# xiyichen/smplify-x-partial

Hardware: AMD Instinct MI355X
Metric: fitted frames/sec (higher is better)
Workload: dtype f32; 1 GPU; configs[1]: 256 synthetic frames/GPU, body-only K=25, camera + 5-stage L-BFGS (fit_smplx_smplifyx.yaml, use_vposer=False); frames_per_gpu=256, lbs_mode=dense, gemm_columns_per_gpu=256, parallelism=frames sharded, dp1, closure_evals_per_frame_max=4429, non_finite=0

## Files before the change

include/sfx.h:

```cpp
#ifndef SFX_H_
#define SFX_H_
#include <stdint.h>

#ifdef __cplusplus
extern "C" {
#endif

typedef struct sfx_model sfx_model;
typedef struct sfx_batch sfx_batch;

typedef struct sfx_model_desc {
    int32_t V, F, J;
    int32_t num_betas, num_expr;
    int32_t num_pca;
    const float*   v_template;
    const float*   shapedirs;
    const float*   posedirs;
    const float*   J_regressor;
    const float*   lbs_weights;
    const int32_t* parents;
    const float*   hands_comp_l;
    const float*   hands_comp_r;
    const float*   pose_mean;
    const int32_t* faces;
// ... 95 lines not shown
                          const float* reye, const float* pose_embedding,
                          const float* regression_pose);
int  sfx_batch_get_params(sfx_batch* b, float* cam_translation, float* global_orient,
                          float* betas, float* lhand, float* rhand, float* expression,
                          float* jaw, float* leye, float* reye, float* pose_embedding,
                          float* body_pose );

int  sfx_batch_num_vars(sfx_batch* b, int32_t stage);
int  sfx_batch_closure(sfx_batch* b, int32_t stage, float* loss_out, float* grad_out, void* stream);

int  sfx_batch_guess_init(sfx_batch* b, const int32_t* pairs , int32_t n_pairs,
                          void* stream);

int  sfx_batch_fit(sfx_batch* b, int32_t first_stage, int32_t last_stage, void* stream);

int  sfx_batch_step(sfx_batch* b, int32_t stage, int32_t resume, float* loss_out, void* stream);

int  sfx_batch_get_grad(sfx_batch* b, int32_t stage, float* grad_out);

int  sfx_batch_pen_stats(sfx_batch* b, int32_t* stats_host , int32_t* ext_n_host );
int  sfx_batch_pen_flags(sfx_batch* b, int32_t* flags_host);
int  sfx_batch_pen_launches(sfx_batch* b);
int  sfx_batch_pen_pairs(sfx_batch* b, int32_t column, int32_t cap, int32_t* pairs_host, int32_t* n_out);

int  sfx_batch_get_stats(sfx_batch* b, float* stage_loss, int32_t* stage_evals,
                         int32_t* stage_ref_evals);

int  sfx_batch_trace(sfx_batch* b, int32_t capacity);
int  sfx_batch_get_trace(sfx_batch* b, float* records, int32_t* counts);

// ... 55 lines not shown
```

smplify-x-partial_amd/_capi.py:

```python
import ctypes as C
import os

import numpy as np

_HERE = os.path.dirname(os.path.abspath(__file__))
LIB_PATH = os.environ.get("SFX_LIB", os.path.join(_HERE, "libsfx.so"))
_lib = None

f32p = C.POINTER(C.c_float)
i32p = C.POINTER(C.c_int32)
f64p = C.POINTER(C.c_double)


class ModelDesc(C.Structure):
    _fields_ = [
        ("V", C.c_int32), ("F", C.c_int32), ("J", C.c_int32),
        ("num_betas", C.c_int32), ("num_expr", C.c_int32), ("num_pca", C.c_int32),
        ("v_template", f32p), ("shapedirs", f32p), ("posedirs", f32p), ("J_regressor", f32p),
        ("lbs_weights", f32p), ("parents", i32p), ("hands_comp_l", f32p), ("hands_comp_r", f32p),
        ("pose_mean", f32p), ("faces", i32p),
        ("n_extra", C.c_int32), ("extra_vertex_ids", i32p),
        ("n_lmk", C.c_int32), ("lmk_faces_idx", i32p), ("lmk_bary", f32p),
        ("n_dyn_rows", C.c_int32), ("n_dyn", C.c_int32), ("dyn_lmk_faces_idx", i32p), ("dyn_lmk_bary", f32p),
        ("K", C.c_int32), ("joint_map", i32p),
# ... 41 lines not shown
SYMBOLS = {
    "sfx_model_create": (C.c_int, [C.POINTER(ModelDesc), C.POINTER(C.c_void_p)]),
    "sfx_model_destroy": (None, [C.c_void_p]),
    "sfx_model_set_parts": (C.c_int, [C.c_void_p, i32p, i32p, i32p, C.c_int32]),
    "sfx_model_set_vposer": (C.c_int, [C.c_void_p, C.c_int32, C.c_int32] + [f32p] * 6),
    "sfx_lbs_forward": (C.c_int, [C.c_void_p, C.c_int32] + [C.c_void_p] * 12 + [C.c_void_p]),
    "sfx_batch_create": (C.c_int, [C.c_void_p, C.POINTER(BatchCfg), C.POINTER(StageWeights), C.POINTER(C.c_void_p)]),
    "sfx_batch_destroy": (None, [C.c_void_p]),
    "sfx_batch_set_frames": (C.c_int, [C.c_void_p] + [f32p] * 5),
    "sfx_batch_set_params": (C.c_int, [C.c_void_p] + [f32p] * 11),
    "sfx_batch_get_params": (C.c_int, [C.c_void_p] + [f32p] * 11),
    "sfx_batch_num_vars": (C.c_int, [C.c_void_p, C.c_int32]),
    "sfx_batch_closure": (C.c_int, [C.c_void_p, C.c_int32, f32p, f32p, C.c_void_p]),
    "sfx_batch_guess_init": (C.c_int, [C.c_void_p, i32p, C.c_int32, C.c_void_p]),
    "sfx_batch_fit": (C.c_int, [C.c_void_p, C.c_int32, C.c_int32, C.c_void_p]),
    "sfx_batch_step": (C.c_int, [C.c_void_p, C.c_int32, C.c_int32, f32p, C.c_void_p]),
    "sfx_batch_pen_stats": (C.c_int, [C.c_void_p, i32p, i32p]),
    "sfx_batch_get_grad": (C.c_int, [C.c_void_p, C.c_int32, f32p]),
    "sfx_batch_set_stage_weights_f64": (C.c_int, [C.c_void_p, C.POINTER(StageWeights64)]),
    "sfx_batch_set_frames_f64": (C.c_int, [C.c_void_p] + [f64p] * 5),
    "sfx_batch_set_params_f64": (C.c_int, [C.c_void_p] + [f64p] * 11),
    "sfx_batch_get_params_f64": (C.c_int, [C.c_void_p] + [f64p] * 11),
    "sfx_batch_closure_f64": (C.c_int, [C.c_void_p, C.c_int32, f64p, f64p, C.c_void_p]),
    "sfx_batch_get_grad_f64": (C.c_int, [C.c_void_p, C.c_int32, f64p]),
    "sfx_batch_get_stats": (C.c_int, [C.c_void_p, f32p, i32p, i32p]),
    "sfx_lbfgs_two_loop": (C.c_int, [C.c_void_p, C.c_void_p, C.c_int32, C.c_int32, C.c_void_p, C.c_void_p]),
    "sfx_batch_trace": (C.c_int, [C.c_void_p, C.c_int32]),
    "sfx_batch_get_trace": (C.c_int, [C.c_void_p, f32p, i32p]),
    "sfx_batch_forward": (C.c_int, [C.c_void_p, C.c_void_p, C.c_void_p, C.c_void_p]),
    "sfx_pen_create": (C.c_int, [C.c_int32, C.c_int32, i32p, i32p, i32p, i32p, C.c_int32, C.c_int32, C.c_int32,
# ... 111 lines not shown
```

smplify-x-partial_amd/csrc/api.hip:

```cpp
#include "../../include/sfx.h"
#include "sfx_internal.h"
#include "model_tables.h"

#include <algorithm>
#include <chrono>
#include <cmath>
#include <cstdarg>
#include <cstdio>
#include <cstring>
#include <map>
#include <memory>
#include <mutex>
#include <string>
#include <vector>

static thread_local char g_err[1024] = "";
void sfx_set_error(const char* fmt, ...) {
    va_list ap; va_start(ap, fmt); vsnprintf(g_err, sizeof(g_err), fmt, ap); va_end(ap);
}
extern "C" const char* sfx_last_error(void) { return g_err; }
extern "C" const char* sfx_version(void) { return "sfx 0.1.0 (gfx950)"; }

struct ProfAcc { double ms = 0; int64_t n = 0, seen = 0; double units = 0; std::vector<std::pair<hipEvent_t, hipEvent_t>> pend; };
static int g_prof = 0;
// ... 83 lines not shown
    DevModel M{};
    DevAlloc mem;
    std::vector<int> faces_host, segm_host, parents_host, ign_host;
    int NB = 0, NE = 0, NPCA = 0;
    std::vector<int> meta_host;
    sfx_batch* fwd = nullptr;
    int fwd_B = 0;
    sfx_pen* pen_idle = nullptr;
    int pen_idle_cols = 0, pen_idle_cap = 0, pen_idle_gen = -1;
    int parts_gen = 0;
    std::mutex pen_mu;
    ~sfx_model() { sfx_batch_destroy(fwd); sfx_pen_destroy(pen_idle); }
};

#define SFX_POLL_BUFS 8
struct sfx_batch {
    sfx_model* m = nullptr;
    BatchDev D{};
    DevAlloc mem;
    VarList* vl_dev = nullptr;
    StageW* sw_dev = nullptr;
    VarList vl_host[2];
    int* stage_host = nullptr;
    int* map_host = nullptr;
    int* act_dev = nullptr;
    int* act_new_dev = nullptr;
    int slots = 0;
    hipEvent_t poll_ev[SFX_POLL_BUFS] = {};
    std::vector<int> slot_host;
    int K = 0;
    sfx_pen* pen = nullptr;
    float pen_sigma = 0.f; int pen_outside = 1;
    int pen_cols = 0, pen_cap = 0, pen_gen = -1;
    std::map<int, hipGraphExec_t> pen_graphs;
    int pen_graph_nodes = 0;
    hipStream_t cap_stream = nullptr;
    int* pen_stats_all = nullptr;
    bool pen_chunked = false;
    bool f64 = false;
    StageW64* sw64_dev = nullptr;
    DevAlloc trace_mem;
    long long* dbg_buf = nullptr;
    ~sfx_batch() {
        for (auto& kv : pen_graphs) hipGraphExecDestroy(kv.second);
        if (cap_stream) hipStreamDestroy(cap_stream);
        if (pen) {
            (void)hipDeviceSynchronize();
            std::lock_guard<std::mutex> lk(m->pen_mu);
            if (pen_gen == m->parts_gen && (!m->pen_idle || m->pen_idle_cols <= pen_cols)) {
                sfx_pen_destroy(m->pen_idle);
                m->pen_idle = pen; m->pen_idle_cols = pen_cols; m->pen_idle_cap = pen_cap; m->pen_idle_gen = pen_gen;
            } else sfx_pen_destroy(pen);
        }
        if (stage_host) hipHostFree(stage_host);
        if (map_host) hipHostFree(map_host);
        for (hipEvent_t e : poll_ev) if (e) hipEventDestroy(e);
    }
};

static int refuse_f64(const sfx_batch* b, const char* fn) {
// ... 41 lines not shown
    M.J_template = mem.up(T.J_template); M.J_dirs = mem.up(T.J_dirs);
    M.J_template64 = mem.up(T.J_template64); M.J_dirs64 = mem.up(T.J_dirs64);
    M.comp_l = mem.up(d->hands_comp_l, (size_t)d->num_pca * SFX_NHAND); M.comp_r = mem.up(d->hands_comp_r, (size_t)d->num_pca * SFX_NHAND);
    M.pose_mean = mem.up(d->pose_mean, SFX_POSE);
    M.sj_start = mem.up(T.sj_start); M.sj_item = mem.up(T.sj_item); M.sj_w = mem.up(T.sj_w);
    M.dj_start = mem.up(T.dj_start); M.dj_item = mem.up(T.dj_item); M.dj_w = mem.up(T.dj_w);
    M.dynp_vid = mem.up(T.dynp_vid); M.dynp_w = mem.up(T.dynp_w); M.dynp_vt = mem.up(T.dynp_vt);
    M.dynp_wj = mem.up(T.dynp_wj); M.dynp_ww = mem.up(T.dynp_ww);
    M.dynp_js = T.dynp_js.empty() ? nullptr : mem.up(T.dynp_js);
    M.dynp_ji = mem.up(T.dynp_ji); M.dynp_jw = mem.up(T.dynp_jw);
    M.item_vid = mem.up(T.item_vid); M.item_w = mem.up(T.item_w);
    M.item_vt = mem.up(T.item_vt); M.item_wj = mem.up(T.item_wj); M.item_ww = mem.up(T.item_ww);
    M.dynp_us = T.dynp_us.empty() ? nullptr : mem.up(T.dynp_us);
    M.vslot = mem.up(T.vslot); M.item_uslot = mem.up(T.item_uslot);
    M.meta = mem.up(T.meta);
    m->meta_host = std::move(T.meta); m->faces_host = std::move(T.faces);
    if (mem.failed) { (void)hipGetLastError(); sfx_set_error("out of device memory (model constants)"); return -2; }
    if (hipDeviceSynchronize() != hipSuccess) { sfx_set_error("model upload failed"); return -2; }
    *out = m.release();
    return 0;
}

extern "C" void sfx_model_destroy(sfx_model* m) { delete m; }

extern "C" int sfx_model_set_parts(sfx_model* m, const int32_t* segm, const int32_t* parents, const int32_t* ign_pairs,
                                   int32_t n_ign) {
    if (!m) { sfx_set_error("null argument"); return -1; }
    { std::lock_guard<std::mutex> lk(m->pen_mu); ++m->parts_gen; if (m->pen_idle) { sfx_pen_destroy(m->pen_idle); m->pen_idle = nullptr; } }
    if (!segm && !parents) {
        m->segm_host.clear(); m->parents_host.clear(); m->ign_host.clear();
// ... 137 lines not shown
        D.cam64 = b->mem.zeros<double>((size_t)B * 8);
    }
    D.gt = b->mem.zeros<float>((size_t)B * K * 2);
    D.conf = b->mem.zeros<float>((size_t)B * K);
    D.jw = b->mem.zeros<float>((size_t)B * K);
    D.cmask = b->mem.zeros<float>((size_t)B * K);
    D.cam = b->mem.zeros<float>((size_t)B * 8);
    D.camR = b->mem.zeros<float>((size_t)B * 9);
    D.regpose = b->mem.zeros<float>((size_t)B * 63);
    D.fd = b->mem.zeros<float>((size_t)B * FD_N);
    D.f = b->mem.zeros<float>(B);
    D.g = b->mem.zeros<float>((size_t)B * SFX_NVAR_MAX);
    D.bodypose = b->mem.zeros<float>((size_t)B * 63);
    D.featR = b->mem.zeros<float>((size_t)SFX_KD_PAD * D.Bpad);
    D.AT = b->mem.zeros<float>((size_t)12 * SFX_JPAD * D.Bpad);
    D.verts = b->mem.zeros<float>((size_t)B * m->M.V * 3);
    D.fwd = b->mem.zeros<float>((size_t)B * SFX_FWD_N);
    D.uvp = b->mem.zeros<float>((size_t)B * std::max(1, m->M.n_uniq) * 3);
    if (D.cfg.pen) {
        const int F = (int)(m->faces_host.size() / 3);
        const bool parts = !m->segm_host.empty();
        const int pen_cols = (c->slots > 0 && c->slots < B && c->lbs_mode == 1) ? std::min(B, ((c->slots + 31) / 32) * 32) : B;
        const int pen_cap = std::max(1, c->max_collisions);
        {
            std::lock_guard<std::mutex> lk(m->pen_mu);
            if (m->pen_idle && m->pen_idle_cols >= pen_cols && m->pen_idle_cap == pen_cap && m->pen_idle_gen == m->parts_gen) {
                b->pen = m->pen_idle; b->pen_cols = m->pen_idle_cols;
                m->pen_idle = nullptr;
                sfx_pen_reuse(b->pen);
            } else if (m->pen_idle) { sfx_pen_destroy(m->pen_idle); m->pen_idle = nullptr; }
// ... 34 lines not shown
    D.stage_loss = b->mem.zeros<float>((size_t)B * (1 + SFX_MAX_STAGES));
    D.stage_evals = b->mem.zeros<int>((size_t)B * (1 + SFX_MAX_STAGES));
    D.stage_ref_evals = b->mem.zeros<int>((size_t)B * (1 + SFX_MAX_STAGES));
    D.X0 = b->mem.zeros<float>((size_t)B * SFX_NPAR_MAX);
    D.gocam = b->mem.zeros<float>((size_t)B * 4);
    D.stage_loss2 = b->mem.zeros<float>((size_t)B * (1 + SFX_MAX_STAGES));
    D.try_both = b->mem.zeros<int>(B);
    D.orient_pass = b->mem.zeros<int>(B);
    if (b->mem.failed) { (void)hipGetLastError(); sfx_set_error("out of device memory (batch of %d frames)", B); return -2; }
    if (hipHostMalloc((void**)&b->stage_host, (size_t)SFX_POLL_BUFS * B * sizeof(int)) != hipSuccess) b->stage_host = nullptr;
    if (hipHostMalloc((void**)&b->map_host, (size_t)SFX_POLL_BUFS * 3 * B * sizeof(int)) != hipSuccess) b->map_host = nullptr;
    if (c->lbs_mode == 1 && (!b->stage_host || !b->map_host)) {
        sfx_set_error("out of pinned host memory"); return -2; }
    for (int i = 0; i < SFX_POLL_BUFS; ++i)
        if (hipEventCreateWithFlags(&b->poll_ev[i], hipEventDisableTiming) != hipSuccess) { sfx_set_error("event creation failed"); return -2; }
    *out = b.release();
    return 0;
}

extern "C" void sfx_batch_destroy(sfx_batch* b) { delete b; }

__global__ void k_pack_fd(BatchDev D, int K) {
    const int b = blockIdx.x, t = threadIdx.x;
    float* fd = D.fd + (size_t)b * FD_N;
    for (int i = t; i < 2 * K; i += blockDim.x) fd[FD_GT + i] = D.gt[(size_t)b * K * 2 + i];
    for (int i = t; i < K; i += blockDim.x) {
        fd[FD_CONF + i] = D.conf[(size_t)b * K + i]; fd[FD_JW + i] = D.jw[(size_t)b * K + i]; fd[FD_CMASK + i] = D.cmask[(size_t)b * K + i]; }
    if (t < 8) fd[FD_CAM + t] = D.cam[(size_t)b * 8 + t];
    if (t < 9) fd[FD_CAMR + t] = D.camR[(size_t)b * 9 + t];
    if (t < 63) fd[FD_REG + t] = D.regpose[(size_t)b * 63 + t];
}
static void pack_fd(sfx_batch* b, hipStream_t s) {
    hipLaunchKernelGGL(k_pack_fd, dim3(b->D.cfg.B), dim3(128), 0, s, b->D, b->K);
}

// ... 450 lines not shown
        auto upload = [&](const std::vector<int>* fresh) -> int {
            int* h = b->map_host + (size_t)upl * 3 * B; upl = (upl + 1) % SFX_POLL_BUFS;
            memcpy(h, col.data(), (size_t)B * sizeof(int));
            memcpy(h + B, run.data(), run.size() * sizeof(int));
            SFX_CHECK(hipMemcpyAsync(D.slot, h, (size_t)B * sizeof(int), hipMemcpyHostToDevice, s));
            if (!run.empty()) SFX_CHECK(hipMemcpyAsync(b->act_dev, h + B, run.size() * sizeof(int), hipMemcpyHostToDevice, s));
            if (fresh && !fresh->empty()) {
                memcpy(h + 2 * B, fresh->data(), fresh->size() * sizeof(int));
                SFX_CHECK(hipMemcpyAsync(b->act_new_dev, h + 2 * B, fresh->size() * sizeof(int), hipMemcpyHostToDevice, s));
            }
            D.act = b->act_dev; D.nrun = (int)run.size();
            return 0;
        };
        D.nact = pool;
        if (int rc = upload(nullptr)) return rc;
        { ProfScope p("tick", s, D.nrun); launch_tick_dense(M, D, b->vl_dev, b->sw_dev, first_stage, last_stage, 0, s); }
        double host_enq_s = 0.0, host_wait_s = 0.0; long host_batches = 0;
        const double wall0 = std::chrono::duration<double>(std::chrono::steady_clock::now().time_since_epoch()).count();
        const int rpb = std::max(1, std::min(64, rpb_env > 0 ? rpb_env : 8));
        auto rounds = [&](int buf) -> int {
            if (dbg_nact) nact_hist[std::min(8, (D.nact - 1) / 32)] += rpb;
            const auto h0 = std::chrono::steady_clock::now();
            struct HostClock { const std::chrono::steady_clock::time_point t0; double& acc; long& n; bool on;
                               ~HostClock() { if (on) { acc += std::chrono::duration<double>(std::chrono::steady_clock::now() - t0).count(); ++n; } } } hc{h0, host_enq_s, host_batches, true};
            for (int q = 0; q < rpb; ++q, ++tick) {
                { ProfScope p("lbs_dense", s, D.nact); launch_lbs_dense(M, D, s); }
                if (int rc = eval_penetration(b, -2, s, true)) return rc;
                ProfScope p("tick", s, D.nrun);
                launch_tick_dense(M, D, b->vl_dev, b->sw_dev, first_stage, last_stage, 1, s);
            }
            SFX_CHECK(hipMemcpyAsync(b->stage_host + (size_t)buf * B, D.stage, (size_t)B * sizeof(int), hipMemcpyDeviceToHost, s));
            SFX_CHECK(hipEventRecord(b->poll_ev[buf], s));
            return 0;
        };
        const int ahead = std::max(1, std::min(SFX_POLL_BUFS - 1, ahead_env > 0 ? ahead_env : (b->pen ? 1 : 3)));
        long q_head = 0, q_next = 0;
        for (; q_next < ahead; ++q_next) if (int rc = rounds((int)(q_next % SFX_POLL_BUFS))) return rc;
        while (!done && tick < max_ticks + (long)rpb * (ahead + 1)) {
            if (int rc = rounds((int)(q_next % SFX_POLL_BUFS))) return rc;
            ++q_next;
            const int cur = (int)(q_head % SFX_POLL_BUFS); ++q_head;
            {
                const auto w0 = std::chrono::steady_clock::now();
                SFX_CHECK(hipEventSynchronize(b->poll_ev[cur]));
// ... 5 lines not shown
            bool changed = false;
            for (size_t r = 0; r < run.size(); ++r) {
                const int f = run[r];
                if (hq[f] <= last_stage) { run[w++] = f; continue; }
                changed = true;
                const int c = col[f];
                col[f] = -1;
                if (next_q < B) { const int nf = next_q++; col[nf] = c; fresh.push_back(nf); }
            }
            run.resize(w);
            for (int nf : fresh) run.push_back(nf);
            done = run.empty();
            if (!done && changed) {
                if (!fresh.empty()) {
                    if (int rc = upload(&fresh)) return rc;
                    BatchDev Dn = D; Dn.act = b->act_new_dev; Dn.nrun = (int)fresh.size();
                    ProfScope p("tick_admit", s, Dn.nrun);
                    launch_tick_dense(M, Dn, b->vl_dev, b->sw_dev, first_stage, last_stage, 0, s);
                } else if ((D.nact + 31) / 32 != ((int)run.size() + 31) / 32 || (D.nact > 16 && run.size() <= 16)) {
                    int q = 0;
                    for (int f : run) col[f] = q++;
                    D.nact = q;
                    if (int rc = upload(nullptr)) return rc;
                    ProfScope p("tick", s, D.nrun);
                    launch_tick_dense(M, D, b->vl_dev, b->sw_dev, first_stage, last_stage, 0, s);
                } else {
                    if (int rc = upload(nullptr)) return rc;
                }
            }
        }
        SFX_CHECK(hipStreamSynchronize(s));
        D.act = nullptr; D.nrun = 0;
        const double wall = std::chrono::duration<double>(std::chrono::steady_clock::now().time_since_epoch()).count() - wall0;
        {
            std::lock_guard<std::mutex> lk(g_prof_mu);
            g_loop_host[0] += host_enq_s; g_loop_host[1] += host_wait_s; g_loop_host[2] += wall; g_loop_host[3] += (double)host_batches * rpb;
        }
        if (dbg_host) {
            fprintf(stderr, "[sfx] host enqueue: %ld batches of rounds, %.1f us of host time per round, %.1f %% of the loop's %.1f ms wall time\n",
                    host_batches, 1e6 * host_enq_s / std::max(1L, host_batches * rpb), 100.0 * host_enq_s / std::max(wall, 1e-9), 1e3 * wall);
        }
        if (dbg_nact) {
            fprintf(stderr, "[sfx] rounds by active columns (<=32, <=64, ..., <=256, more), cumulative:");
            for (int i = 0; i < 9; ++i) fprintf(stderr, " %ld", nact_hist[i]);
            fprintf(stderr, "\n");
// ... 288 lines not shown
```

smplify-x-partial_amd/csrc/lbs_dense.hip:

```cpp
#include "sfx_internal.h"
#include <cstdlib>
#include <algorithm>

typedef float f32x4 __attribute__((ext_vector_type(4)));

#define DT 256
#ifndef KC
#define KC 32
#endif
#ifndef MINW
#define MINW 3
#endif
#define FB 128
#define VB 16
#define NB3 (VB * 3)
#define LDK (KC + 4)
#define LDB NB3
#define B4 (KC * NB3 / 4)

#define MFMA(a, b, c) __builtin_amdgcn_mfma_f32_16x16x4f32((a), (b), (c), 0, 0, 0)

#define KCHUNK(c) (((c) + 1) % NCHUNK)

#ifdef SFX_LAB
#include "lbs_dense_lab.h"
#endif

#define FB3 64
template <int W>
struct __align__(16) DenseLDS16 {
    float a[2][16 * W][LDK];
    float b[2][KC][LDB];
};
#ifndef MINW16
#define MINW16 4
#endif
template <int W>
__global__ __launch_bounds__(64 * W, MINW16)
void k_lbs_dense16(DevModel M, BatchDev D) {
    constexpr int DTW = 64 * W, FBW = 16 * W;
    static_assert(W >= 3 && W <= 8, "staging: two rounds of DTW threads cover the 384 float4 of a dirs chunk");
    __shared__ DenseLDS16<W> S;
    const int tid = threadIdx.x;
    const int lane = tid & 63, wv = tid >> 6;
    int tile, fblk, fpb;
    {
        const int ny = (D.nact + FBW - 1) / FBW, ntile = (M.V + VB - 1) / VB;
        const int tpx = (ntile + 7) / 8;
        const int L = blockIdx.x, xcd = L & 7, slot = L >> 3;
        tile = xcd * tpx + slot / ny; fblk = slot % ny;
        if (tile >= ntile) return;
        fpb = 16 * (((D.nact + 15) / 16 + ny - 1) / ny);
    }
    const int v0 = tile * VB;
    const int fb0 = fblk * fpb;
    const int b0 = fb0 + wv * 16;
    const int jl = lane & 15, kq = lane >> 4;
    const int V = M.V, B = D.nact;
    const int vtx = v0 + jl;
    const int v = vtx < V ? vtx : V - 1;
    const size_t Bp = (size_t)D.Bpad;
    const size_t LD = (size_t)3 * M.Vpad;
    const bool active = wv * 16 < fpb && b0 < B;
    const float4* gA = reinterpret_cast<const float4*>(D.featR + (size_t)fb0 * SFX_KD_PAD);
    const float4* gB = reinterpret_cast<const float4*>(M.dirs_tiled + (size_t)tile * SFX_KD_PAD * NB3);
    const int stepA = KC / 4, stepB = KC * (NB3 / 4);
// ... 89 lines not shown
    if (vok) {
#pragma unroll
        for (int r = 0; r < 4; ++r) {
            const int f0 = b0 + kq * 4 + r;
            if (f0 < B) { float* o = D.verts + ((size_t)f0 * V + vtx) * 3; o[0] = o0[r][0]; o[1] = o0[r][1]; o[2] = o0[r][2]; }
        }
    }
}

struct __align__(16) DenseLDS16c {
    float a[2][32][LDK];
    float b[2][KC][LDB];
    float x[2][3][64][4];
};
__global__ __launch_bounds__(384, 2)
void k_lbs_dense16c(DevModel M, BatchDev D) {
    __shared__ DenseLDS16c S;
    const int tid = threadIdx.x;
    const int lane = tid & 63, wv = tid >> 6, sl = wv / 3, co = wv % 3;
    int tile;
    {
        const int ntile = (M.V + VB - 1) / VB, tpx = (ntile + 7) / 8;
        const int L = blockIdx.x, xcd = L & 7, slot = L >> 3;
        tile = xcd * tpx + slot;
        if (tile >= ntile || slot >= tpx) return;
    }
    const int v0 = tile * VB, b0 = sl * 16;
    const int jl = lane & 15, kq = lane >> 4;
    const int V = M.V, B = D.nact;
    const int vtx = v0 + jl;
    const int v = vtx < V ? vtx : V - 1;
    const size_t Bp = (size_t)D.Bpad;
    const bool active = b0 < B;
    const float4* gA = reinterpret_cast<const float4*>(D.featR);
    const float4* gB = reinterpret_cast<const float4*>(M.dirs_tiled + (size_t)tile * SFX_KD_PAD * NB3);
    const int stepA = KC / 4, stepB = KC * (NB3 / 4);
    const bool okA = tid < 32 * (KC / 4);
    const int ia = okA ? tid : 0, fa = ia / (KC / 4), ka = ia % (KC / 4);
    const int gAo = (min(fa, D.Bpad - 1)) * (SFX_KD_PAD / 4) + ka, lAo = fa * LDK + ka * 4;
    const int gBo = tid, lBo = (tid / (NB3 / 4)) * LDB + (tid % (NB3 / 4)) * 4;
// ... 69 lines not shown
                if (D.vposed) D.vposed[((size_t)f0 * V + vtx) * 3 + co] = co == 0 ? ax0[r] : co == 1 ? ay0[r] : az0[r];
                D.verts[((size_t)f0 * V + vtx) * 3 + co] = o0[r];
            }
        }
    }
}


#ifdef SFX_LAB
int g_lbs_dense_form = [] { const char* e = getenv("SFX_LBS_DENSE"); return e ? atoi(e) : 16; }();
static int g_lbs_dense_w = [] { const char* e = getenv("SFX_LBS_W"); const int v = e ? atoi(e) : 0; return (v >= 3 && v <= 5) ? v : 0; }();
#else
constexpr int g_lbs_dense_form = 16, g_lbs_dense_w = 0;
#endif

void launch_lbs_dense(const DevModel& M, const BatchDev& D, hipStream_t s) {
    if (D.nact <= 0) return;
#ifdef MF32
    {
        const int ny = (D.nact + FB - 1) / FB, ntile = (M.V + VB2 - 1) / VB2;
        dim3 grid(8 * ((ntile + 7) / 8) * ny);
        hipLaunchKernelGGL(k_lbs_dense32, grid, dim3(DT), 0, s, M, D);
        return;
    }
#endif
#ifdef SFX_LAB
    if (g_lbs_dense_form == 32) {
        const int ny = (D.nact + FB - 1) / FB, ntile = (M.V + VB - 1) / VB;
        hipLaunchKernelGGL(k_lbs_dense, dim3(8 * ((ntile + 7) / 8) * ny), dim3(DT), 0, s, M, D);
        return;
    }
#endif
    {
        const int ns = (D.nact + 15) / 16, ny4 = (ns + 3) / 4;
        if (ns <= 2 && g_lbs_dense_form != 17 && !g_lbs_dense_w) {
            const int ntile_ = (M.V + VB - 1) / VB;
            hipLaunchKernelGGL(k_lbs_dense16c, dim3(8 * ((ntile_ + 7) / 8)), dim3(384), 0, s, M, D);
            return;
        }
        int w = ns <= 4 ? 4 : (ns == 5 ? 5 : std::max(3, (ns + ny4 - 1) / ny4));
        if (g_lbs_dense_w) w = g_lbs_dense_w;
        const int ny = (ns + w - 1) / w, ntile = (M.V + VB - 1) / VB;
        dim3 grid(8 * ((ntile + 7) / 8) * ny);
        switch (w) {
        case 3: hipLaunchKernelGGL(k_lbs_dense16<3>, grid, dim3(192), 0, s, M, D); break;
        case 5: hipLaunchKernelGGL(k_lbs_dense16<5>, grid, dim3(320), 0, s, M, D); break;
        default: hipLaunchKernelGGL(k_lbs_dense16<4>, grid, dim3(256), 0, s, M, D); break;
        }
    }
}
```

smplify-x-partial_amd/csrc/model_tables.h:

```cpp
#pragma once
#include "../../include/sfx.h"
#include "sfx_internal.h"
#include <algorithm>
#include <cstring>
#include <vector>

struct ModelTables {
    int Vpad = 0, n_rounds = 0, n_items = 0, n_static_items = 0, n_uniq = 0, n_sj = 0, n_dyn_items = 0;
#ifdef SFX_LAB
    std::vector<float> dirs;
#endif
    std::vector<float> dirs_tiled, dirsT, tj_w, jv_w, Wsp_w, J_template, J_dirs, item_w, item_vt, item_ww, sj_w, dj_w;
    std::vector<float> dynp_w, dynp_vt, dynp_ww, dynp_jw;
    std::vector<double> J_template64, J_dirs64;
    std::vector<int> tj_n, tj_list, jv_start, jv_vid, Wsp_j, vslot, item_uslot, item_vid, item_wj, sj_start, sj_item;
    std::vector<int> dj_start, dj_item, dynp_vid, dynp_wj, dynp_js, dynp_ji, dynp_us;
    std::vector<int> meta;
    std::vector<int> faces;
};

static inline void sfx_pack_weights(const float* W, int v, int* wj, float* ww) {
    int n = 0;
    for (int j = 0; j < SFX_J; ++j) {
        const float w = W[(size_t)v * SFX_J + j];
        if (w == 0.f) continue;
        if (n < SFX_NW) { wj[n] = j; ww[n] = w; }
        ++n;
    }
    if (n > SFX_NW) wj[0] = -1;
}
static inline int sfx_dyn_vertex(const sfx_model_desc* d, int row, int l, int c) {
    return d->faces[(size_t)d->dyn_lmk_faces_idx[(size_t)row * d->n_dyn + l] * 3 + c];
// ... 127 lines not shown
    }
    const int nt = T.Vpad / 16;
    T.tj_n.assign(nt, 0); T.tj_list.assign((size_t)nt * SFX_JPAD, 0); T.tj_w.assign((size_t)nt * SFX_JPAD * 16, 0.f);
    for (int t = 0; t < nt; ++t) {
        int n = 0;
        for (int j = 0; j < SFX_J; ++j) {
            bool used = false;
            for (int q = 0; q < 16 && !used; ++q) { const int v = t * 16 + q; used = v < V && W[(size_t)v * SFX_J + j] != 0.f; }
            if (!used) continue;
            T.tj_list[(size_t)t * SFX_JPAD + n] = j;
            for (int q = 0; q < 16; ++q) { const int v = t * 16 + q; T.tj_w[((size_t)t * SFX_JPAD + n) * 16 + q] = v < V ? W[(size_t)v * SFX_J + j] : 0.f; }
            ++n;
        }
        T.tj_n[t] = ((n + 3) / 4) * 4;
    }
    T.J_template64.resize((size_t)SFX_J * 3); T.J_dirs64.resize((size_t)SFX_J * 3 * S);
    for (int j = 0; j < SFX_J; ++j) {
        std::vector<double> acc(3 + 3 * S, 0.0);
        const float* jr = d->J_regressor + (size_t)j * V;
        for (int v = 0; v < V; ++v) {
            const double w = jr[v];
            if (w == 0.0) continue;
            for (int c = 0; c < 3; ++c) {
                acc[c] += w * d->v_template[(size_t)v * 3 + c];
                const float* sd = d->shapedirs + ((size_t)v * 3 + c) * S;
                for (int l = 0; l < S; ++l) acc[3 + c * S + l] += w * sd[l];
            }
        }
        std::copy_n(acc.begin(), 3, &T.J_template64[(size_t)j * 3]); std::copy_n(acc.begin() + 3, 3 * S, &T.J_dirs64[(size_t)j * 3 * S]);
    }
// ... 6 lines not shown
```

smplify-x-partial_amd/csrc/sfx_internal.h:

```cpp
#pragma once
#include <hip/hip_runtime.h>
#include <stdint.h>
#include <algorithm>
#include <vector>

#define SFX_J 55
#define SFX_POSE (3 * SFX_J)
#define SFX_NHAND 45
#define SFX_MAX_K 144
#define SFX_MAX_ITEMS 240
#define SFX_SMALL_ITEMS 32
#define SFX_MAX_DYN 64
#ifndef SFX_RIF_BIG
#define SFX_RIF_BIG 8
#endif
#ifndef SFX_RIF_SMALL
#define SFX_RIF_SMALL 9
#endif
#ifndef SFX_SMALL_OCC
#define SFX_SMALL_OCC 1
#endif
#define SFX_KD_PAD 512
#define SFX_JPAD 56
#define SFX_MAX_LEVELS 16
// ... 67 lines not shown
#endif
    const float* dirs_tiled;
    const float* dirsT;
    const float* W;
    const void*  gap6_;
    const int*   tj_n;
    const int*   tj_list;
    const float* tj_w;
    const int*   jv_start;
    const int*   jv_vid;
    const float* jv_w;
    const int*   Wsp_j;
    const float* Wsp_w;
    const float* J_template;
    const float* J_dirs;
    const void*  gap7_[4];
    const float* comp_l;
    const float* comp_r;
    const float* pose_mean;
    const void*  gap8_[7];
    int n_items, n_static_items;
    int n_uniq;
    const int* vslot;
    const int* item_uslot;
    const int*   item_vid;
    const float* item_w;
    const float* item_vt;
    const int*   item_wj;
    const float* item_ww;
    const void*  gap9_[4];
    int Vpad;
// ... 156 lines not shown
}
void launch_closure(const DevModel& M, const BatchDev& D, const VarList* vl_dev, const StageW* sw_dev,
                    const ClosureArgs& a, hipStream_t s);
void launch_closure64(const DevModel& M, const BatchDev& D, const VarList* vl_dev, const StageW64* sw_dev,
                      const ClosureArgs& a, hipStream_t s);
struct PenAdjPrep {
    const float* AT;
    const int*   Wsp_j;
    const float* Wsp_w;
    const float* W;
    float*       adj_G;
    int Bpad, Vpad;
};
void launch_pen_adjoint(const DevModel& M, const BatchDev& D, hipStream_t s);
int sfx_adj_slices(const DevModel& M);
void launch_lbs_dense(const DevModel& M, const BatchDev& D, hipStream_t s);
#ifdef SFX_LAB
extern int g_lbs_dense_form;
#endif
void launch_lbfgs_tick(const DevModel& M, const BatchDev& D, const VarList* vl_dev, int first_stage,
                       int last_stage, int init, int step_mode, hipStream_t s);
size_t sfx_optstate_size();
int debug_two_loop(const float* S, const float* Y, int cnt, int hist_cap, const float* g, float* d_out);
void launch_fit_rows(const DevModel& M, const BatchDev& D, const VarList* vl_dev, const StageW* sw_dev,
                     int first_stage, int last_stage, int max_ticks, hipStream_t s);
void launch_tick_dense(const DevModel& M, const BatchDev& D, const VarList* vl_dev, const StageW* sw_dev,
                       int first_stage, int last_stage, int has_eval, hipStream_t s);
```

smplify-x-partial_amd/engine.py:

```python
import ctypes as C

import numpy as np

from . import _capi as capi
from .synthetic import SMPLX_EXTRA_VERTEX_IDS

NUM_BODY_JOINTS = {"coco25": 25, "halpe": 26, "coco_wholebody": 23}
PARAM_NAMES = ("cam_translation", "global_orient", "betas", "left_hand_pose", "right_hand_pose",
               "expression", "jaw_pose", "leye_pose", "reye_pose", "pose_embedding")


def _jaw_weights(cfg, shape_weights):
    jw = cfg.get("jaw_pose_prior_weights")
    if jw is None:
        return [[x] * 3 for x in shape_weights]
    return [[float(v) for v in e.split(",")] if isinstance(e, str) else [float(v) for v in e] for e in jw]


def stage_weights_from_cfg(cfg, struct=None):
    use_hands, use_face = cfg.get("use_hands", True), cfg.get("use_face", True)
    bpw = cfg.get("body_pose_prior_weights") or [4.04 * 1e2, 4.04 * 1e2, 57.4, 4.78]
    n = len(bpw)
    lists = {"data": cfg.get("data_weights") or [1] * n, "bpw": bpw,
             "shape": cfg.get("shape_weights") or [1e2, 5 * 1e1, 1e1, .5 * 1e1]}
# ... 322 lines not shown
            capi.check(self._lib.sfx_batch_closure_f64(self._h, stage, capi.dptr(loss), capi.dptr(grad), None))
            return loss, grad
        loss = np.zeros(self.B, np.float32)
        grad = np.zeros((self.B, N), np.float32)
        capi.check(self._lib.sfx_batch_closure(self._h, stage, capi.fptr(loss), capi.fptr(grad), None))
        return loss, grad

    def guess_init(self, pairs):
        p = capi.i32(np.asarray(pairs).reshape(-1, 2))
        capi.check(self._lib.sfx_batch_guess_init(self._h, capi.iptr(p), p.shape[0], None))

    def fit(self, first_stage=-1, last_stage=None, stream=None):
        last = self.n_stages - 1 if last_stage is None else last_stage
        capi.check(self._lib.sfx_batch_fit(self._h, first_stage, last, C.c_void_p(stream) if stream else None))

    def step(self, stage, resume):
        loss = np.zeros(self.B, np.float32)
        capi.check(self._lib.sfx_batch_step(self._h, stage, int(bool(resume)), capi.fptr(loss), None))
        return loss

    def set_gmm(self, prior):
        mu = np.ascontiguousarray(prior.means.detach().cpu().numpy(), np.float32)
        P = np.ascontiguousarray(prior.precisions.detach().cpu().numpy(), np.float32)
        nw = np.ascontiguousarray(prior.nll_weights.detach().cpu().numpy().reshape(-1), np.float32)
        cc = None
        if not getattr(prior, "use_merged", True):
            import torch
            cov_term = torch.log(torch.det(prior.covs) + prior.epsilon)
            cc = np.ascontiguousarray((0.5 * (cov_term + prior.random_var_dim * prior.pi_term)).detach().cpu().numpy().reshape(-1), np.float32)
        capi.check(self._lib.sfx_batch_set_gmm_form(self._h, mu.shape[0], mu.shape[1], capi.fptr(mu), capi.fptr(P), capi.fptr(nw),
# ... 223 lines not shown
```

Baseline: 569.4 frames/s.

## Split dense LBS into item and rest tiles, overlapping rest on side stream

Measured after the change: 522.0 frames/s. 8.3% lower.

```diff
diff --git a/include/sfx.h b/include/sfx.h
--- a/include/sfx.h
+++ b/include/sfx.h
@@ -133,6 +133,8 @@
 
 int  sfx_batch_fit(sfx_batch* b, int32_t first_stage, int32_t last_stage, void* stream);
 
+int  sfx_batch_set_overlap(sfx_batch* b, int32_t max_running);
+
 int  sfx_batch_step(sfx_batch* b, int32_t stage, int32_t resume, float* loss_out, void* stream);
 
 int  sfx_batch_get_grad(sfx_batch* b, int32_t stage, float* grad_out);
diff --git a/smplify-x-partial_amd/_capi.py b/smplify-x-partial_amd/_capi.py
--- a/smplify-x-partial_amd/_capi.py
+++ b/smplify-x-partial_amd/_capi.py
@@ -79,6 +79,7 @@
     "sfx_batch_closure": (C.c_int, [C.c_void_p, C.c_int32, f32p, f32p, C.c_void_p]),
     "sfx_batch_guess_init": (C.c_int, [C.c_void_p, i32p, C.c_int32, C.c_void_p]),
     "sfx_batch_fit": (C.c_int, [C.c_void_p, C.c_int32, C.c_int32, C.c_void_p]),
+    "sfx_batch_set_overlap": (C.c_int, [C.c_void_p, C.c_int32]),
     "sfx_batch_step": (C.c_int, [C.c_void_p, C.c_int32, C.c_int32, f32p, C.c_void_p]),
     "sfx_batch_pen_stats": (C.c_int, [C.c_void_p, i32p, i32p]),
     "sfx_batch_get_grad": (C.c_int, [C.c_void_p, C.c_int32, f32p]),
diff --git a/smplify-x-partial_amd/csrc/api.hip b/smplify-x-partial_amd/csrc/api.hip
--- a/smplify-x-partial_amd/csrc/api.hip
+++ b/smplify-x-partial_amd/csrc/api.hip
@@ -121,6 +121,8 @@
 };
 
 #define SFX_POLL_BUFS 8
+#define SFX_OVERLAP_DEFAULT 128
+#define SFX_OV_EVS 8
 struct sfx_batch {
     sfx_model* m = nullptr;
     BatchDev D{};
@@ -134,6 +136,10 @@
     int* act_new_dev = nullptr;
     int slots = 0;
     hipEvent_t poll_ev[SFX_POLL_BUFS] = {};
+    hipStream_t side_stream = nullptr;
+    hipEvent_t ov_ev[SFX_OV_EVS] = {};
+    float* featR2 = nullptr; float* AT2 = nullptr;
+    int overlap_max = -1;
     std::vector<int> slot_host;
     int K = 0;
     sfx_pen* pen = nullptr;
@@ -151,6 +157,8 @@
     ~sfx_batch() {
         for (auto& kv : pen_graphs) hipGraphExecDestroy(kv.second);
         if (cap_stream) hipStreamDestroy(cap_stream);
+        if (side_stream) { (void)hipStreamSynchronize(side_stream); hipStreamDestroy(side_stream); }
+        for (hipEvent_t e : ov_ev) if (e) hipEventDestroy(e);
         if (pen) {
             (void)hipDeviceSynchronize();
             std::lock_guard<std::mutex> lk(m->pen_mu);
@@ -222,6 +230,8 @@
     M.dynp_us = T.dynp_us.empty() ? nullptr : mem.up(T.dynp_us);
     M.vslot = mem.up(T.vslot); M.item_uslot = mem.up(T.item_uslot);
     M.meta = mem.up(T.meta);
+    M.tl_items = mem.up(T.tl_items); M.tl_rest = mem.up(T.tl_rest);
+    M.tl_items_n = (int)T.tl_items.size(); M.tl_rest_n = (int)T.tl_rest.size();
     m->meta_host = std::move(T.meta); m->faces_host = std::move(T.faces);
     if (mem.failed) { (void)hipGetLastError(); sfx_set_error("out of device memory (model constants)"); return -2; }
     if (hipDeviceSynchronize() != hipSuccess) { sfx_set_error("model upload failed"); return -2; }
@@ -389,6 +399,10 @@
     D.bodypose = b->mem.zeros<float>((size_t)B * 63);
     D.featR = b->mem.zeros<float>((size_t)SFX_KD_PAD * D.Bpad);
     D.AT = b->mem.zeros<float>((size_t)12 * SFX_JPAD * D.Bpad);
+    if (c->lbs_mode == 1 && !D.cfg.pen && D.cfg.n_stages > 0 && m->M.tl_items_n > 0 && m->M.tl_rest_n > 0) {
+        b->featR2 = b->mem.zeros<float>((size_t)SFX_KD_PAD * D.Bpad);
+        b->AT2 = b->mem.zeros<float>((size_t)12 * SFX_JPAD * D.Bpad);
+    }
     D.verts = b->mem.zeros<float>((size_t)B * m->M.V * 3);
     D.fwd = b->mem.zeros<float>((size_t)B * SFX_FWD_N);
     D.uvp = b->mem.zeros<float>((size_t)B * std::max(1, m->M.n_uniq) * 3);
@@ -453,11 +467,23 @@
         sfx_set_error("out of pinned host memory"); return -2; }
     for (int i = 0; i < SFX_POLL_BUFS; ++i)
         if (hipEventCreateWithFlags(&b->poll_ev[i], hipEventDisableTiming) != hipSuccess) { sfx_set_error("event creation failed"); return -2; }
+    if (b->featR2) {
+        if (hipStreamCreateWithFlags(&b->side_stream, hipStreamNonBlocking) != hipSuccess) { b->side_stream = nullptr; sfx_set_error("stream creation failed"); return -2; }
+        for (int i = 0; i < SFX_OV_EVS; ++i)
+            if (hipEventCreateWithFlags(&b->ov_ev[i], hipEventDisableTiming) != hipSuccess) { sfx_set_error("event creation failed"); return -2; }
+    }
     *out = b.release();
     return 0;
 }
 
 extern "C" void sfx_batch_destroy(sfx_batch* b) { delete b; }
+
+extern "C" int sfx_batch_set_overlap(sfx_batch* b, int32_t max_running) {
+    if (!b) { sfx_set_error("null batch"); return -1; }
+    if (max_running < -1) { sfx_set_error("max_running %d: -1 (built-in threshold), 0 (never split) or a frame count", max_running); return -1; }
+    b->overlap_max = max_running;
+    return 0;
+}
 
 __global__ void k_pack_fd(BatchDev D, int K) {
     const int b = blockIdx.x, t = threadIdx.x;
@@ -938,6 +964,21 @@
         };
         D.nact = pool;
         if (int rc = upload(nullptr)) return rc;
+        float* const fbuf[2] = {D.featR, b->featR2}; float* const abuf[2] = {D.AT, b->AT2};
+        const int split_max = !(b->featR2 && b->side_stream) ? 0 : b->overlap_max < 0 ? SFX_OVERLAP_DEFAULT : b->overlap_max;
+        const bool dbuf = split_max > 0;
+        hipStream_t side = b->side_stream;
+        hipEvent_t rest_ev = nullptr;
+        long n_eval = 0; int ov_i = 0;
+        struct SideJoin {
+            BatchDev& D; float* f0; float* a0; hipStream_t side; bool on;
+            ~SideJoin() { if (on) (void)hipStreamSynchronize(side); D.featR = f0; D.AT = a0; }
+        } side_join{D, fbuf[0], abuf[0], side, dbuf};
+        auto operands = [&](long e) { if (dbuf) { D.featR = fbuf[e & 1]; D.AT = abuf[e & 1]; } };
+        auto join_rest = [&]() -> int {
+            if (rest_ev) { SFX_CHECK(hipStreamWaitEvent(s, rest_ev, 0)); rest_ev = nullptr; }
+            return 0;
+        };
         { ProfScope p("tick", s, D.nrun); launch_tick_dense(M, D, b->vl_dev, b->sw_dev, first_stage, last_stage, 0, s); }
         double host_enq_s = 0.0, host_wait_s = 0.0; long host_batches = 0;
         const double wall0 = std::chrono::duration<double>(std::chrono::steady_clock::now().time_since_epoch()).count();
@@ -948,10 +989,24 @@
             struct HostClock { const std::chrono::steady_clock::time_point t0; double& acc; long& n; bool on;
                                ~HostClock() { if (on) { acc += std::chrono::duration<double>(std::chrono::steady_clock::now() - t0).count(); ++n; } } } hc{h0, host_enq_s, host_batches, true};
             for (int q = 0; q < rpb; ++q, ++tick) {
-                { ProfScope p("lbs_dense", s, D.nact); launch_lbs_dense(M, D, s); }
+                if (dbuf && D.nrun <= split_max) {
+                    { ProfScope p("lbs_dense", s, D.nact); launch_lbs_dense(M, D, s, LBS_ITEMS); }
+                    hipEvent_t ei = b->ov_ev[ov_i], er = b->ov_ev[ov_i + 1]; ov_i = (ov_i + 2) % SFX_OV_EVS;
+                    SFX_CHECK(hipEventRecord(ei, s));
+                    SFX_CHECK(hipStreamWaitEvent(side, ei, 0));
+                    { ProfScope p("lbs_rest", side, D.nact); launch_lbs_dense(M, D, side, LBS_REST); }
+                    SFX_CHECK(hipEventRecord(er, side));
+                    if (int rc = join_rest()) return rc;
+                    rest_ev = er;
+                } else {
+                    if (int rc = join_rest()) return rc;
+                    ProfScope p("lbs_dense", s, D.nact); launch_lbs_dense(M, D, s);
+                }
                 if (int rc = eval_penetration(b, -2, s, true)) return rc;
                 ProfScope p("tick", s, D.nrun);
+                operands(n_eval + 1);
                 launch_tick_dense(M, D, b->vl_dev, b->sw_dev, first_stage, last_stage, 1, s);
+                ++n_eval;
             }
             SFX_CHECK(hipMemcpyAsync(b->stage_host + (size_t)buf * B, D.stage, (size_t)B * sizeof(int), hipMemcpyDeviceToHost, s));
             SFX_CHECK(hipEventRecord(b->poll_ev[buf], s));
@@ -987,6 +1042,7 @@
             if (!done && changed) {
                 if (!fresh.empty()) {
                     if (int rc = upload(&fresh)) return rc;
+                    if (int rc = join_rest()) return rc;
                     BatchDev Dn = D; Dn.act = b->act_new_dev; Dn.nrun = (int)fresh.size();
                     ProfScope p("tick_admit", s, Dn.nrun);
                     launch_tick_dense(M, Dn, b->vl_dev, b->sw_dev, first_stage, last_stage, 0, s);
@@ -995,6 +1051,7 @@
                     for (int f : run) col[f] = q++;
                     D.nact = q;
                     if (int rc = upload(nullptr)) return rc;
+                    if (int rc = join_rest()) return rc;
                     ProfScope p("tick", s, D.nrun);
                     launch_tick_dense(M, D, b->vl_dev, b->sw_dev, first_stage, last_stage, 0, s);
                 } else {
@@ -1002,6 +1059,7 @@
                 }
             }
         }
+        if (int rc = join_rest()) return rc;
         SFX_CHECK(hipStreamSynchronize(s));
         D.act = nullptr; D.nrun = 0;
         const double wall = std::chrono::duration<double>(std::chrono::steady_clock::now().time_since_epoch()).count() - wall0;
diff --git a/smplify-x-partial_amd/csrc/lbs_dense.hip b/smplify-x-partial_amd/csrc/lbs_dense.hip
--- a/smplify-x-partial_amd/csrc/lbs_dense.hip
+++ b/smplify-x-partial_amd/csrc/lbs_dense.hip
@@ -37,7 +37,7 @@
 #endif
 template <int W>
 __global__ __launch_bounds__(64 * W, MINW16)
-void k_lbs_dense16(DevModel M, BatchDev D) {
+void k_lbs_dense16(DevModel M, BatchDev D, const int* __restrict__ tiles, int ntl) {
     constexpr int DTW = 64 * W, FBW = 16 * W;
     static_assert(W >= 3 && W <= 8, "staging: two rounds of DTW threads cover the 384 float4 of a dirs chunk");
     __shared__ DenseLDS16<W> S;
@@ -48,8 +48,15 @@
         const int ny = (D.nact + FBW - 1) / FBW, ntile = (M.V + VB - 1) / VB;
         const int tpx = (ntile + 7) / 8;
         const int L = blockIdx.x, xcd = L & 7, slot = L >> 3;
-        tile = xcd * tpx + slot / ny; fblk = slot % ny;
-        if (tile >= ntile) return;
+        if (tiles) {
+            const int tpl = ntl >> 3, q = slot / ny;
+            tile = q < tpl ? tiles[xcd * tpl + q] : -1;
+            if (tile < 0 || tile >= ntile) return;
+        } else {
+            tile = xcd * tpx + slot / ny;
+            if (tile >= ntile) return;
+        }
+        fblk = slot % ny;
         fpb = 16 * (((D.nact + 15) / 16 + ny - 1) / ny);
     }
     const int v0 = tile * VB;
@@ -169,7 +176,7 @@
     float x[2][3][64][4];
 };
 __global__ __launch_bounds__(384, 2)
-void k_lbs_dense16c(DevModel M, BatchDev D) {
+void k_lbs_dense16c(DevModel M, BatchDev D, const int* __restrict__ tiles, int ntl) {
     __shared__ DenseLDS16c S;
     const int tid = threadIdx.x;
     const int lane = tid & 63, wv = tid >> 6, sl = wv / 3, co = wv % 3;
@@ -177,8 +184,14 @@
     {
         const int ntile = (M.V + VB - 1) / VB, tpx = (ntile + 7) / 8;
         const int L = blockIdx.x, xcd = L & 7, slot = L >> 3;
-        tile = xcd * tpx + slot;
-        if (tile >= ntile || slot >= tpx) return;
+        if (tiles) {
+            const int tpl = ntl >> 3;
+            tile = slot < tpl ? tiles[xcd * tpl + slot] : -1;
+            if (tile < 0 || tile >= ntile) return;
+        } else {
+            tile = xcd * tpx + slot;
+            if (tile >= ntile || slot >= tpx) return;
+        }
     }
     const int v0 = tile * VB, b0 = sl * 16;
     const int jl = lane & 15, kq = lane >> 4;
@@ -278,9 +291,13 @@
 constexpr int g_lbs_dense_form = 16, g_lbs_dense_w = 0;
 #endif
 
-void launch_lbs_dense(const DevModel& M, const BatchDev& D, hipStream_t s) {
+void launch_lbs_dense(const DevModel& M, const BatchDev& D, hipStream_t s, LbsTiles which) {
     if (D.nact <= 0) return;
+    const int* tiles = which == LBS_ITEMS ? M.tl_items : which == LBS_REST ? M.tl_rest : nullptr;
+    const int ntl = which == LBS_ITEMS ? M.tl_items_n : which == LBS_REST ? M.tl_rest_n : 0;
+    if (which != LBS_ALL && ntl == 0) return;
 #ifdef MF32
+    if (which == LBS_REST) return;
     {
         const int ny = (D.nact + FB - 1) / FB, ntile = (M.V + VB2 - 1) / VB2;
         dim3 grid(8 * ((ntile + 7) / 8) * ny);
@@ -290,6 +307,7 @@
 #endif
 #ifdef SFX_LAB
     if (g_lbs_dense_form == 32) {
+        if (which == LBS_REST) return;
         const int ny = (D.nact + FB - 1) / FB, ntile = (M.V + VB - 1) / VB;
         hipLaunchKernelGGL(k_lbs_dense, dim3(8 * ((ntile + 7) / 8) * ny), dim3(DT), 0, s, M, D);
         return;
@@ -299,17 +317,17 @@
         const int ns = (D.nact + 15) / 16, ny4 = (ns + 3) / 4;
         if (ns <= 2 && g_lbs_dense_form != 17 && !g_lbs_dense_w) {
             const int ntile_ = (M.V + VB - 1) / VB;
-            hipLaunchKernelGGL(k_lbs_dense16c, dim3(8 * ((ntile_ + 7) / 8)), dim3(384), 0, s, M, D);
+            hipLaunchKernelGGL(k_lbs_dense16c, dim3(tiles ? ntl : 8 * ((ntile_ + 7) / 8)), dim3(384), 0, s, M, D, tiles, ntl);
             return;
         }
         int w = ns <= 4 ? 4 : (ns == 5 ? 5 : std::max(3, (ns + ny4 - 1) / ny4));
         if (g_lbs_dense_w) w = g_lbs_dense_w;
         const int ny = (ns + w - 1) / w, ntile = (M.V + VB - 1) / VB;
-        dim3 grid(8 * ((ntile + 7) / 8) * ny);
+        dim3 grid((tiles ? ntl : 8 * ((ntile + 7) / 8)) * ny);
         switch (w) {
-        case 3: hipLaunchKernelGGL(k_lbs_dense16<3>, grid, dim3(192), 0, s, M, D); break;
-        case 5: hipLaunchKernelGGL(k_lbs_dense16<5>, grid, dim3(320), 0, s, M, D); break;
-        default: hipLaunchKernelGGL(k_lbs_dense16<4>, grid, dim3(256), 0, s, M, D); break;
+        case 3: hipLaunchKernelGGL(k_lbs_dense16<3>, grid, dim3(192), 0, s, M, D, tiles, ntl); break;
+        case 5: hipLaunchKernelGGL(k_lbs_dense16<5>, grid, dim3(320), 0, s, M, D, tiles, ntl); break;
+        default: hipLaunchKernelGGL(k_lbs_dense16<4>, grid, dim3(256), 0, s, M, D, tiles, ntl); break;
         }
     }
 }
diff --git a/smplify-x-partial_amd/csrc/model_tables.h b/smplify-x-partial_amd/csrc/model_tables.h
--- a/smplify-x-partial_amd/csrc/model_tables.h
+++ b/smplify-x-partial_amd/csrc/model_tables.h
@@ -16,6 +16,7 @@
     std::vector<int> tj_n, tj_list, jv_start, jv_vid, Wsp_j, vslot, item_uslot, item_vid, item_wj, sj_start, sj_item;
     std::vector<int> dj_start, dj_item, dynp_vid, dynp_wj, dynp_js, dynp_ji, dynp_us;
     std::vector<int> meta;
+    std::vector<int> tl_items, tl_rest;
     std::vector<int> faces;
 };
 
@@ -173,6 +174,22 @@
         }
         T.tj_n[t] = ((n + 3) / 4) * 4;
     }
+    {
+        const int ntile = (V + 15) / 16, tpx = (ntile + 7) / 8;
+        std::vector<int> rows_i[8], rows_r[8];
+        for (int t = 0, ni_t = 0; t < ntile; ++t) {
+            bool item = false;
+            for (int q = 0; q < 16 && !item; ++q) item = T.vslot[t * 16 + q] >= 0;
+            if (item) rows_i[ni_t++ % 8].push_back(t); else rows_r[t / tpx].push_back(t);
+        }
+        auto pack = [](const std::vector<int>* rows, std::vector<int>& out_) {
+            size_t n = 0;
+            for (int x = 0; x < 8; ++x) n = std::max(n, rows[x].size());
+            out_.assign(8 * n, -1);
+            for (int x = 0; x < 8; ++x) std::copy(rows[x].begin(), rows[x].end(), out_.begin() + x * n);
+        };
+        pack(rows_i, T.tl_items); pack(rows_r, T.tl_rest);
+    }
     T.J_template64.resize((size_t)SFX_J * 3); T.J_dirs64.resize((size_t)SFX_J * 3 * S);
     for (int j = 0; j < SFX_J; ++j) {
         std::vector<double> acc(3 + 3 * S, 0.0);
diff --git a/smplify-x-partial_amd/csrc/sfx_internal.h b/smplify-x-partial_amd/csrc/sfx_internal.h
--- a/smplify-x-partial_amd/csrc/sfx_internal.h
+++ b/smplify-x-partial_amd/csrc/sfx_internal.h
@@ -105,7 +105,10 @@
     const float* Wsp_w;
     const float* J_template;
     const float* J_dirs;
-    const void*  gap7_[4];
+    const int*   tl_items;
+    const int*   tl_rest;
+    int tl_items_n, tl_rest_n;
+    const void*  gap7_;
     const float* comp_l;
     const float* comp_r;
     const float* pose_mean;
@@ -292,7 +295,8 @@
 };
 void launch_pen_adjoint(const DevModel& M, const BatchDev& D, hipStream_t s);
 int sfx_adj_slices(const DevModel& M);
-void launch_lbs_dense(const DevModel& M, const BatchDev& D, hipStream_t s);
+enum LbsTiles { LBS_ALL = 0, LBS_ITEMS, LBS_REST };
+void launch_lbs_dense(const DevModel& M, const BatchDev& D, hipStream_t s, LbsTiles which = LBS_ALL);
 #ifdef SFX_LAB
 extern int g_lbs_dense_form;
 #endif
diff --git a/smplify-x-partial_amd/engine.py b/smplify-x-partial_amd/engine.py
--- a/smplify-x-partial_amd/engine.py
+++ b/smplify-x-partial_amd/engine.py
@@ -360,6 +360,9 @@
         last = self.n_stages - 1 if last_stage is None else last_stage
         capi.check(self._lib.sfx_batch_fit(self._h, first_stage, last, C.c_void_p(stream) if stream else None))
 
+    def set_overlap(self, max_running=-1):
+        capi.check(self._lib.sfx_batch_set_overlap(self._h, int(max_running)))
+
     def step(self, stage, resume):
         loss = np.zeros(self.B, np.float32)
         capi.check(self._lib.sfx_batch_step(self._h, stage, int(bool(resume)), capi.fptr(loss), None))
```
